# PFLeget/treegp

Measured on AMD Instinct MI355X. Metric: GP solve+predict throughput, 2-D AnisotropicRBF N=65536, higher is better.
Workload: dtype f64

## Files before the change

### include/tgp.h

```cpp
#ifndef TGP_H
#define TGP_H

#include <stdint.h>

#ifdef __cplusplus
extern "C" {
#endif

typedef struct tgp_ctx tgp_ctx;
typedef struct tgp_factor tgp_factor;

enum {
    TGP_RBF = 0,
    TGP_ARBF = 1,
    TGP_VK = 2,
    TGP_AVK = 3
};

typedef struct {
    int32_t kind;
    int32_t _pad;
    double amp;
    double a, b, c;
    double ell;
// ... 143 lines not shown
int tgp_dd_update2(tgp_ctx *ctx, double *d_Aloc, const int64_t *d_loff, int64_t Np, int kpanel, int G, int g,
                   const double *d_gathered0, int cmax0, const double *d_gathered1, int cmax1, int col_lo,
                   int col_hi);
int tgp_dd_update_group(tgp_ctx *ctx, double *d_Aloc, const int64_t *d_loff, int64_t Np, int kpanel, int G, int g,
                        int nseg, const double *const *d_gathered, const int *cmax, int col_lo, int col_hi);
int tgp_dd_strip_left(tgp_ctx *ctx, double *d_Aloc, const int64_t *h_loff, const int64_t *d_loff, int64_t Np, int kgroup, int b,
                      int G, int g, const double *d_ext);
int tgp_dd_queue_reset(tgp_ctx *ctx);
int tgp_dd_set_exclusive(tgp_ctx *ctx, int on);
int tgp_dd_update_group_queued(tgp_ctx *ctx, double *d_Aloc, const int64_t *d_loff, int64_t Np, int kpanel, int G, int g,
                               int nseg, const double *const *d_gathered, const int *cmax, int col_lo, int col_hi, int nres);
int tgp_dd_update_group_fused(tgp_ctx *ctx, double *d_Aloc, const int64_t *d_loff, int64_t Np, int kpanel, int G, int g, int nseg,
                              const double *const *d_gathered, const int *cmax, int head_cols, int nres);
int tgp_dd_wait_head(tgp_ctx *ctx, tgp_ctx *waiter);
int tgp_dd_tail_assemble(tgp_ctx *ctx, const double *d_gathered, int64_t stride, int64_t Np, int k0, int G, double *d_tail);
int tgp_dd_tail_scatter(tgp_ctx *ctx, const double *d_tail, int64_t Np, int k0, int G, int g, double *d_Aloc, const int64_t *d_loff);
int tgp_handoff_mode(tgp_ctx *ctx);
int tgp_dd_keep_panel(tgp_ctx *ctx, double *d_Afull, int64_t Np, int kpanel, int G, const double *d_bcast,
                      const double *d_gathered, int cmax);
int tgp_dd_fwd_diag(tgp_ctx *ctx, const double *d_Aloc, const int64_t *h_loff, int kb, const double *d_W, double *d_yk);
int tgp_dd_fwd_update(tgp_ctx *ctx, const double *d_Aloc, const int64_t *h_loff, int64_t Np, int kb, int G, int g,
                      const double *d_zk, double *d_yloc);
int tgp_dd_bwd_partial(tgp_ctx *ctx, const double *d_Aloc, const int64_t *h_loff, int64_t Np, int kb, int G, int g,
                       const double *d_aloc, double *d_s);
int tgp_dd_bwd_diag(tgp_ctx *ctx, const double *d_Aloc, const int64_t *h_loff, int kb, const double *d_W, double *d_ak,
                    const double *d_s );
int tgp_dd_logdet_local(tgp_ctx *ctx, const double *d_Aloc, const int64_t *d_loff, int64_t Np, int64_t n, int G, int g,
                        double *d_out);
int tgp_dd_info(tgp_ctx *ctx, int reset);

int tgp_debug_syrk_loop(tgp_ctx *ctx, double *d_A, int64_t Np, int reps, double *ms_per_launch,
                        double *flops_per_launch);
int tgp_debug_tilemap(int64_t T, int32_t *ti, int32_t *tj, int64_t cap);

#ifdef __cplusplus
}
#endif
#endif
```

### treegp_amd/_lib.py

```python
import ctypes as C
import os
import threading

import numpy as np

_HERE = os.path.dirname(os.path.abspath(__file__))
LIB_PATH = os.environ.get("TGP_LIB_PATH") or os.path.join(_HERE, "csrc", "libtgp.so")

TGP_RBF, TGP_ARBF, TGP_VK, TGP_AVK = 0, 1, 2, 3
NTIMINGS = 12


class TgpKernel(C.Structure):
    _fields_ = [("kind", C.c_int32), ("_pad", C.c_int32), ("amp", C.c_double), ("a", C.c_double),
                ("b", C.c_double), ("c", C.c_double), ("ell", C.c_double)]


_dp = C.POINTER(C.c_double)
_vp = C.c_void_p
_i64 = C.c_int64

SIGNATURES = {
    "tgp_init": (C.c_int, [C.POINTER(C.c_int), C.c_int, C.POINTER(_vp)]),
    "tgp_destroy": (None, [_vp]),
# ... 25 lines not shown
    "tgp_d2h": (C.c_int, [_vp, _vp, _vp, _i64]),
    "tgp_sync": (C.c_int, [_vp]),
    "tgp_stream": (_vp, [_vp]),
    "tgp_mem_info": (C.c_int, [_vp, C.POINTER(_i64), C.POINTER(_i64)]),
    "tgp_d_gp_solve": (C.c_int, [_vp, C.POINTER(TgpKernel), _vp, _i64, _vp, _vp, _vp, _dp, _dp, C.POINTER(_vp)]),
    "tgp_d_gp_predict": (C.c_int, [_vp, C.POINTER(TgpKernel), _vp, _i64, _vp, _vp, _i64, _vp]),
    "tgp_d_gp_predict_grad": (C.c_int, [_vp, C.POINTER(TgpKernel), _vp, _i64, _vp, _vp, _i64, _vp]),
    "tgp_panel_off": (_i64, [_i64, _i64]),
    "tgp_panel_elems": (_i64, [_i64]),
    "tgp_padded_n": (_i64, [_i64]),
    "tgp_d_kbuild_lower": (C.c_int, [_vp, C.POINTER(TgpKernel), _vp, _i64, _vp, _vp]),
    "tgp_d_potrf": (C.c_int, [_vp, _vp, _i64, _vp]),
    "tgp_d_potrs": (C.c_int, [_vp, _vp, _vp, _i64, _vp]),
    "tgp_d_potrs_multi": (C.c_int, [_vp, _vp, _vp, _i64, _vp, C.c_int]),
    "tgp_gp_solve_dense": (C.c_int, [_vp, _vp, _i64, _vp, _vp, _vp, _dp, _dp, C.POINTER(_vp)]),
    "tgp_d_gp_solve_dense": (C.c_int, [_vp, _vp, _i64, _vp, _vp, _vp, _dp, _dp, C.POINTER(_vp)]),
    "tgp_factor_solve": (C.c_int, [_vp, _vp, _vp, C.c_int, _vp]),
    "tgp_factor_lmul": (C.c_int, [_vp, _vp, _vp, C.c_int, _vp]),
    "tgp_factor_inv_diag": (C.c_int, [_vp, _vp, _vp]),
    "tgp_factor_inv_blocks": (C.c_int, [_vp, _vp, _vp, _i64, _vp]),
    "tgp_gp_solve_batch": (C.c_int, [_vp, C.c_int, _vp, _vp, _i64, _vp, _vp, _vp, _vp, _vp, _vp, _vp]),
    "tgp_gp_solve_grad_batch": (C.c_int, [_vp, C.c_int, _vp, _vp, _i64, _vp, _vp, _vp, _vp, _vp, _vp, _vp]),
    "tgp_gp_loo_batch": (C.c_int, [_vp, C.c_int, _vp, _vp, _i64, _vp, _vp, _vp, _vp, _vp, _vp, _vp, _vp]),
    "tgp_gp_posterior_batch": (C.c_int, [_vp, C.c_int, _vp, _vp, _i64, _vp, _vp, _vp, _vp, _i64, _vp, C.c_int, _vp, _vp, _vp, _vp, _vp]),
    "tgp_gp_predict_cov_dense": (C.c_int, [_vp, _vp, _vp, _vp, _i64, _vp]),
    "tgp_gp_predict_var": (C.c_int, [_vp, _vp, C.POINTER(TgpKernel), _vp, _i64, _vp, _i64, _vp]),
    "tgp_gp_predict_var_dense": (C.c_int, [_vp, _vp, _vp, _vp, _i64, _vp]),
    "tgp_gp_loglik_grad": (C.c_int, [_vp, _vp, C.POINTER(TgpKernel), _vp, _i64, _vp, _vp]),
    "tgp_d_gp_solve_grad": (C.c_int, [_vp, C.POINTER(TgpKernel), _vp, _i64, _vp, _vp, _dp, _dp, _vp]),
    "tgp_d_unpack_lower": (C.c_int, [_vp, _vp, _i64, _i64, _vp]),
    "tgp_factor_device": (C.c_int, [_vp, _vp, C.POINTER(_vp), C.POINTER(_vp), C.POINTER(_i64)]),
    "tgp_debug_syrk_loop": (C.c_int, [_vp, _vp, _i64, C.c_int, _dp, _dp]),
    "tgp_debug_tilemap": (C.c_int, [_i64, _vp, _vp, _i64]),
    "tgp_set_stream": (C.c_int, [_vp, _vp]),
    "tgp_reset_stream": (C.c_int, [_vp]),
    "tgp_set_side_stream": (C.c_int, [_vp, _vp]),
    "tgp_dist_panel_rows": (_i64, [_i64, _i64, C.c_int, C.c_int]),
    "tgp_dist_panel_off": (_i64, [_i64, _i64, C.c_int, C.c_int]),
    "tgp_dist_local_elems": (_i64, [_i64, C.c_int, C.c_int]),
    "tgp_dd_kbuild": (C.c_int, [_vp, C.POINTER(TgpKernel), _vp, _i64, _vp, _vp, _vp, C.c_int, C.c_int]),
    "tgp_dd_factor_diag": (C.c_int, [_vp, _vp, _vp, _i64, C.c_int, C.c_int, C.c_int, _vp, _vp]),
    "tgp_dd_trsm": (C.c_int, [_vp, _vp, _vp, _i64, C.c_int, C.c_int, C.c_int, _vp, _vp]),
    "tgp_dd_update": (C.c_int, [_vp, _vp, _vp, _i64, C.c_int, C.c_int, C.c_int, _vp, C.c_int, C.c_int, C.c_int]),
    "tgp_dd_update2": (C.c_int, [_vp, _vp, _vp, _i64, C.c_int, C.c_int, C.c_int, _vp, C.c_int, _vp, C.c_int, C.c_int, C.c_int]),
    "tgp_dd_update_group": (C.c_int, [_vp, _vp, _vp, _i64, C.c_int, C.c_int, C.c_int, C.c_int, _vp, _vp, C.c_int, C.c_int]),
    "tgp_dd_strip_left": (C.c_int, [_vp, _vp, _vp, _vp, _i64, C.c_int, C.c_int, C.c_int, C.c_int, _vp]),
    "tgp_dd_update_group_queued": (C.c_int, [_vp, _vp, _vp, _i64, C.c_int, C.c_int, C.c_int, C.c_int, _vp, _vp, C.c_int, C.c_int, C.c_int]),
    "tgp_dd_update_group_fused": (C.c_int, [_vp, _vp, _vp, _i64, C.c_int, C.c_int, C.c_int, C.c_int, _vp, _vp, C.c_int, C.c_int]),
    "tgp_dd_wait_head": (C.c_int, [_vp, _vp]),
    "tgp_handoff_mode": (C.c_int, [_vp]),
    "tgp_dd_tail_assemble": (C.c_int, [_vp, _vp, _i64, _i64, C.c_int, C.c_int, _vp]),
    "tgp_dd_tail_scatter": (C.c_int, [_vp, _vp, _i64, C.c_int, C.c_int, C.c_int, _vp, _vp]),
    "tgp_dd_queue_reset": (C.c_int, [_vp]),
    "tgp_dd_set_exclusive": (C.c_int, [_vp, C.c_int]),
    "tgp_dd_keep_panel": (C.c_int, [_vp, _vp, _i64, C.c_int, C.c_int, _vp, _vp, C.c_int]),
    "tgp_dd_fwd_diag": (C.c_int, [_vp, _vp, _vp, C.c_int, _vp, _vp]),
    "tgp_dd_fwd_update": (C.c_int, [_vp, _vp, _vp, _i64, C.c_int, C.c_int, C.c_int, _vp, _vp]),
    "tgp_dd_bwd_partial": (C.c_int, [_vp, _vp, _vp, _i64, C.c_int, C.c_int, C.c_int, _vp, _vp]),
    "tgp_dd_bwd_diag": (C.c_int, [_vp, _vp, _vp, C.c_int, _vp, _vp, _vp]),
    "tgp_dd_logdet_local": (C.c_int, [_vp, _vp, _vp, _i64, _i64, C.c_int, C.c_int, _vp]),
    "tgp_dd_info": (C.c_int, [_vp, C.c_int]),
}

_lib = None
_ctx = {}
_lock = threading.Lock()
# ... 135 lines not shown
```

### treegp_amd/csrc/chol.hip

```cpp
#include "tgp_internal.h"

#include "gemm_tile.h"
#include "potrf128.h"

#ifdef TGP_POTRF_STAMPS
__device__ unsigned long long tgp_gemm_stamps[1024 * 4];
__device__ int tgp_gemm_stamp_grid = 43;
__device__ unsigned long long tgp_queue_stamps[1024 * 4];
__device__ int tgp_queue_stamp_T = 40;
__device__ unsigned long long tgp_mid_stamps[25 * 8];
__device__ int tgp_mid_stamp_base = 5120;
#define TGP_MID_STAMP(i)                                                                                   \
    do {                                                                                                   \
        if (threadIdx.x == 0 && base == tgp_mid_stamp_base && blockIdx.x < 25) tgp_mid_stamps[blockIdx.x * 8 + (i)] = __builtin_amdgcn_s_memrealtime(); \
    } while (0)
#else
#define TGP_MID_STAMP(i) ((void)0)
#endif

namespace {
template <int MODE, int LDB>
__global__ __launch_bounds__(256, 2) void gemm_col_kernel(const double *A, const double *B, double *C) {
    const int64_t t = blockIdx.x;
    TGP_CHAIN_PRIO();
// ... 151 lines not shown
    const int ri = blockIdx.x;
    const int tj = blockIdx.y;
    if (tj > (ri >> 3) || (ri >> 3) >= T) return;
    TGP_CHAIN_PRIO();
    const int64_t pj = ob + (tj >> 1);
    const int64_t I = (int64_t)TGP_PW * ob + 16 * (int64_t)ri;
    double *C = Abase + panel_off(pj, Np) + (I - pj * TGP_PW) * TGP_PW + (tj & 1) * TGP_TB;
    const int64_t oa = (int64_t)ri * 16 * TGP_PW, obb = (int64_t)tj * TGP_TB * TGP_PW;
    nt_slice_tile<1, TGP_PW, NSEG>(nt_slice_lds_storage(), P0 + oa, TGP_PW, P0 + obb, TGP_PW, C, TGP_PW, NSEG > 1 ? P1 + oa : nullptr,
                                   NSEG > 1 ? P1 + obb : nullptr);
}

template <int NSEG>
__global__ __launch_bounds__(256, 2) void syrk_dtv_kernel(double *Abase, int64_t Np, int ob, int T, int strip, const double *P0,
                                                          const double *P1) {
    int ti, tj;
    if (strip == 0) {
        tilemap(blockIdx.x, T, ti, tj);
        if (ti < 0) return;
    } else {
        tj = (int)(blockIdx.x % strip);
        ti = (int)(blockIdx.x / strip);
        if (ti < tj || ti >= T) return;
    }
    if (strip) TGP_CHAIN_PRIO();
    const int64_t pj = ob + (tj >> 1);
    const int64_t I = (int64_t)TGP_PW * ob + (int64_t)TGP_TB * ti;
    double *C = Abase + panel_off(pj, Np) + (I - pj * TGP_PW) * TGP_PW + (tj & 1) * TGP_TB;
    const int64_t oa = (int64_t)ti * TGP_TB * TGP_PW, obb = (int64_t)tj * TGP_TB * TGP_PW;
    gemm_tile_dtv<4, TGP_PW, NSEG>(P0 + oa, P0 + obb, C, NSEG > 1 ? P1 + oa : nullptr, NSEG > 1 ? P1 + obb : nullptr);
}

template <int NSEG>
__global__ __launch_bounds__(256, 2) void syrk_strip64_kernel(double *Abase, int64_t Np, int ob, int T, int strip, const double *P0,
                                                              const double *P1, int ti_min = 0) {
    const int tj = (int)(blockIdx.x % strip);
    const int th = (int)(blockIdx.x / strip) + 2 * ti_min;
    const int ti = th >> 1;
    if (ti < tj || ti >= T) return;
    TGP_CHAIN_PRIO();
    const int64_t pj = ob + (tj >> 1);
    const int64_t I = (int64_t)TGP_PW * ob + (int64_t)64 * th;
    double *C = Abase + panel_off(pj, Np) + (I - pj * TGP_PW) * TGP_PW + (tj & 1) * TGP_TB;
    const int64_t oa = (int64_t)th * 64 * TGP_PW, obb = (int64_t)tj * TGP_TB * TGP_PW;
    gemm_tile_dtv<4, TGP_PW, NSEG, 1>(P0 + oa, P0 + obb, C, NSEG > 1 ? P1 + oa : nullptr, NSEG > 1 ? P1 + obb : nullptr);
}

template <int NSEG>
__global__ __launch_bounds__(256, 2) void syrk_strip32_kernel(double *Abase, int64_t Np, int ob, int T, int strip, const double *P0,
                                                              const double *P1) {
    const int tj = (int)(blockIdx.x % strip);
    const int tq = (int)(blockIdx.x / strip);
    const int ti = tq >> 2;
    if (ti < tj || ti >= T) return;
    TGP_CHAIN_PRIO();
    const int64_t pj = ob + (tj >> 1);
    const int64_t I = (int64_t)TGP_PW * ob + (int64_t)32 * tq;
    double *C = Abase + panel_off(pj, Np) + (I - pj * TGP_PW) * TGP_PW + (tj & 1) * TGP_TB;
    const int64_t oa = (int64_t)tq * 32 * TGP_PW, obb = (int64_t)tj * TGP_TB * TGP_PW;
    gemm_tile_dtv32<TGP_PW, NSEG>(P0 + oa, P0 + obb, C, NSEG > 1 ? P1 + oa : nullptr, NSEG > 1 ? P1 + obb : nullptr);
}

template <int NSEG>
__global__ __launch_bounds__(256, 2) void syrk_dtv_queue_kernel(double *Abase, int64_t Np, int ob, int T, unsigned entries, unsigned half_from, int nres,
                                                                unsigned *__restrict__ queue, const double *P0, const double *P1, int steal) {
    __shared__ unsigned s_slot;
// ... 67 lines not shown
#endif
    }
}

struct HeadSignal {
    unsigned *done = nullptr, *flag = nullptr;
    unsigned target = 0, seq = 0;
    int nhead = 0;
};
__device__ __forceinline__ void head_done(const HeadSignal &h) {
    asm volatile("s_waitcnt vmcnt(0)" ::: "memory");
    __syncthreads();
    if (threadIdx.x < 64) {
        __builtin_amdgcn_fence(__ATOMIC_RELEASE, "agent");
        if (threadIdx.x == 0) {
            const unsigned old = __hip_atomic_fetch_add(h.done, 1u, __ATOMIC_ACQ_REL, __HIP_MEMORY_SCOPE_AGENT);
            if (old + 1u == h.target) __hip_atomic_store(h.flag, h.seq, __ATOMIC_RELEASE, __HIP_MEMORY_SCOPE_SYSTEM);
        }
    }
}

template <int NSEG>
__global__ __launch_bounds__(256, 2) void syrk_segs_kernel(double *Abase, int64_t Np, int ob, int T, int strip, SegPtrs<NSEG> P) {
    int ti, tj;
    if (strip == 0) {
        tilemap(blockIdx.x, T, ti, tj);
        if (ti < 0) return;
    } else {
        tj = (int)(blockIdx.x % strip);
        ti = (int)(blockIdx.x / strip);
        if (ti < tj || ti >= T) return;
    }
    if (strip) TGP_CHAIN_PRIO();
    const int64_t pj = ob + (tj >> 1);
    const int64_t I = (int64_t)TGP_PW * ob + (int64_t)TGP_TB * ti;
    double *C = Abase + panel_off(pj, Np) + (I - pj * TGP_PW) * TGP_PW + (tj & 1) * TGP_TB;
    const int64_t oa = (int64_t)ti * TGP_TB * TGP_PW, obb = (int64_t)tj * TGP_TB * TGP_PW;
    SegPtrs<NSEG> sp;
#pragma unroll
    for (int s = 0; s < NSEG; ++s) {
        sp.a[s] = P.a[s] + oa;
        sp.b[s] = P.a[s] + obb;
    }
    gemm_tile_dtv_segs<4, TGP_PW, NSEG>(sp, C);
}

template <int NSEG>
struct DistSegs {
    const double *P[NSEG];
    const double *PB[NSEG];
    int cmax[NSEG];
    int frg[NSEG];
};
struct DistMap {
    int start[258];
    int ngroups;
    int qfb;
    unsigned ginv;
    int whole;
    int half_from;
    int nhead, head_cols;
    int head_half;
    HeadSignal hs;
};
__device__ __forceinline__ int div_g(int x, unsigned ginv) { return ginv ? (int)__umulhi((unsigned)x, ginv) : x; }
__device__ __forceinline__ int snake_pos(int q, int r, int G) { return (q & 1) ? G - 1 - r : r; }
// ... 163 lines not shown
        gemm_col_small_kernel<0, TGP_TB><<<8, 256, 0, st>>>(R1, W0, R1);
        if (r2 > 0) {
            if (small) gemm_col_small_kernel<0, TGP_TB><<<r2 * 8, 256, 0, st>>>(R2, W0, R2);
            else gemm_col_kernel<0, TGP_TB><<<r2, 256, 0, st>>>(R2, W0, R2);
        }
        gemm_col_small_kernel<1, TGP_PW><<<8, 256, 0, st>>>(R1, R1, R1 + TGP_TB);
        if (r2 > 0) {
            if (small) gemm_col_small_kernel<1, TGP_PW><<<r2 * 8, 256, 0, st>>>(R2, R1, R2 + TGP_TB);
            else gemm_col_kernel<1, TGP_PW><<<r2, 256, 0, st>>>(R2, R1, R2 + TGP_TB);
        }
        run_potrf128(st, R1 + TGP_TB, TGP_PW, W1, d_info, base + TGP_TB, exclusive, solo);
    } else {
        if (r1 <= small_rows) {
            gemm_col_small_kernel<0, TGP_TB><<<r1 * 8, 256, 0, st>>>(R1, W0, R1);
            gemm_col_small_kernel<1, TGP_PW><<<r1 * 8, 256, 0, st>>>(R1, R1, R1 + TGP_TB);
        } else {
            gemm_col_kernel<0, TGP_TB><<<r1, 256, 0, st>>>(R1, W0, R1);
            gemm_col_kernel<1, TGP_PW><<<r1, 256, 0, st>>>(R1, R1, R1 + TGP_TB);
        }
        run_potrf128(st, R1 + TGP_TB, TGP_PW, W1, d_info, base + TGP_TB, exclusive, solo);
    }
    if (r2 > 0) {
        double *R2 = Pk + (int64_t)TGP_PW * TGP_PW + TGP_TB;
        if (r2 <= small_rows) gemm_col_small_kernel<0, TGP_TB><<<r2 * 8, 256, 0, st>>>(R2, W1, R2);
        else gemm_col_kernel<0, TGP_TB><<<r2, 256, 0, st>>>(R2, W1, R2);
    }
}

inline int small_t() {
    static const int v = [] { const char *e = getenv("TGP_SMALL_T"); return e ? atoi(e) : 8; }();
    return v;
}

template <int NSEG>
void launch_syrk(hipStream_t st, double *d_A, int64_t Np, int ob, int T, int strip, const double *P0, const double *P1) {
    if (T <= 0) return;
    static const int strip_small_t = [] { const char *e = getenv("TGP_STRIP_SMALL_T"); return e ? atoi(e) : 16; }();
    if (T <= small_t() || (strip > 0 && T <= strip_small_t)) {
        const int cols = strip == 0 ? T : (strip < T ? strip : T);
        syrk_small_kernel<NSEG><<<dim3((unsigned)(T * 8), (unsigned)cols), 256, 0, st>>>(d_A, Np, ob, T, P0, P1);
        return;
    }
    static const int strip64_t = [] { const char *e = getenv("TGP_STRIP64_T"); return e ? atoi(e) : 128; }();
    static const int strip32_t = [] { const char *e = getenv("TGP_STRIP32_T"); return e ? atoi(e) : 64; }();
    if (strip > 0 && T <= strip32_t) {
        syrk_strip32_kernel<NSEG><<<(unsigned)((int64_t)4 * T * strip), 256, 0, st>>>(d_A, Np, ob, T, strip, P0, P1);
        return;
    }
    if (strip > 0 && T <= strip64_t) {
        syrk_strip64_kernel<NSEG><<<(unsigned)((int64_t)2 * T * strip), 256, 0, st>>>(d_A, Np, ob, T, strip, P0, P1);
        return;
    }
    const unsigned gs = strip == 0 ? (unsigned)tilemap_grid(T) : (unsigned)((int64_t)T * strip);
    syrk_dtv_kernel<NSEG><<<gs, 256, 0, st>>>(d_A, Np, ob, T, strip, P0, P1);
}

int queued_nres(int T) {
    static const int queue_res = [] { const char *e = getenv("TGP_QUEUE_RES"); return e ? atoi(e) : 0; }();
    if (queue_res > 0) return queue_res > TGP_QUEUE_MAXRES ? TGP_QUEUE_MAXRES : queue_res;
    static const int t1 = [] { const char *e = getenv("TGP_QUEUE_T1"); return e ? atoi(e) : 42; }();
    static const int t2 = [] { const char *e = getenv("TGP_QUEUE_T2"); return e ? atoi(e) : 26; }();
    return T >= t1 ? 1 : (T >= t2 ? 2 : 3);
}
void launch_syrk2_queued(tgp_ctx *ctx, hipStream_t st, double *d_A, int64_t Np, int ob, int T, const double *P0, const double *P1,
                         int nqueue) {
    const int nres = queued_nres(T);
    static const int half_env = [] { const char *e = getenv("TGP_QUEUE_HALF"); return e ? atoi(e) : -1; }();
    const unsigned slots = (unsigned)(tilemap_grid(T) / 8);
    unsigned nhalf = half_env >= 0 ? (unsigned)half_env : (unsigned)(512 - 64 * nres) / 8u;
    if (nhalf > slots) nhalf = slots;
    static const int steal = [] { const char *e = getenv("TGP_QUEUE_STEAL"); return e ? atoi(e) : 1; }();
    syrk_dtv_queue_kernel<2><<<512 + 8, 256, 0, st>>>(d_A, Np, ob, T, slots + nhalf, slots - nhalf, nres,
                                                     ctx->d_queue + TGP_QUEUE_WORDS * nqueue, P0, P1, steal);
}
}

int launch_potrf(tgp_ctx *ctx, double *d_A, int64_t Np, double *d_W, bool defer_info, int64_t n_data) {
    TGP_ARG(Np > 0 && Np % TGP_PW == 0);
    hipStream_t st = ctx->stream;
    TGP_HIP(hipMemsetAsync(ctx->d_info, 0, sizeof(int), st));
    const int nP = (int)(Np / TGP_PW);
    const bool prof = ctx->profiling != 0;
    if (prof) {
        while ((int)ctx->prof_events.size() < 2 * nP) {
            hipEvent_t e;
            TGP_HIP(hipEventCreate(&e));
// ... 22 lines not shown
        return 0;
    };
    auto Wk = [&](int k) { return d_W + (int64_t)(2 * k) * TGP_TB * TGP_TB; };
    auto panel = [&](int k) { return d_A + panel_off(k, Np); };
    static const int queue_t = [] { const char *e = getenv("TGP_QUEUE_T"); return e ? atoi(e) : 64; }();
    int nqueue = 0;
    static const bool mid_env = [] { const char *e = getenv("TGP_PANEL_MID"); return e ? atoi(e) != 0 : true; }();
    const bool mid_on = mid_env && !ctx->mid_off && ctx->mid_allowed;
    if (mid_on) TGP_HIP(hipMemsetAsync(ctx->d_psync, 0, (size_t)(nP < TGP_PSYNC_PANELS ? nP : TGP_PSYNC_PANELS) * PANEL_SYNC_WORDS * sizeof(unsigned), st));
    if (Np / TGP_TB - 8 > small_t())
        TGP_HIP(hipMemsetAsync(ctx->d_queue, 0, TGP_NQUEUE * TGP_QUEUE_WORDS * sizeof(unsigned), st));
    auto psync = [&](int k) { return (mid_on && k < TGP_PSYNC_PANELS) ? ctx->d_psync + PANEL_SYNC_WORDS * k : nullptr; };
    auto run_pairs = [&](int kstart) -> int {
        hipStream_t sd = ctx->side_stream;
        auto factor_pair = [&](hipStream_t s, int k, bool exclusive = false, int cus = 0, bool tell = false) {
            const int64_t mk = Np - (int64_t)TGP_PW * k;
            auto sync = [&](int kk) { return (cus > 0 && mid_on && kk < TGP_PSYNC_PANELS) ? ctx->d_psync + PANEL_SYNC_WORDS * kk : nullptr; };
            factor_panel(s, panel(k), mk, Wk(k), ctx->d_info, k * TGP_PW, exclusive, n_data, sync(k), cus);
            if (tell) (void)tgp_signal(ctx, s, 2, ctx->ev[6]);
            if (k + 1 >= nP) return;
            const int T1 = (int)((mk - TGP_PW) / TGP_TB);
            launch_syrk<1>(s, d_A, Np, k + 1, T1, 2, panel(k) + (int64_t)TGP_PW * TGP_PW, nullptr);
            factor_panel(s, panel(k + 1), mk - TGP_PW, Wk(k + 1), ctx->d_info, (k + 1) * TGP_PW, exclusive, n_data, sync(k + 1), cus);
        };
        factor_pair(st, kstart, false, 256);
        static const int split_t = [] { const char *e = getenv("TGP_U2A_SPLIT_T"); return e ? atoi(e) : 64; }();
        bool early = false;
        for (int k = kstart; k + 2 < nP; k += 2) {
            const int T2 = (int)((Np - (int64_t)TGP_PW * (k + 2)) / TGP_TB);
            const double *P0 = panel(k) + (int64_t)2 * TGP_PW * TGP_PW;
            const double *P1 = panel(k + 1) + (int64_t)TGP_PW * TGP_PW;
            const int T3 = T2 - 4;
            const bool queued = T3 <= queue_t && T3 > small_t() && nqueue < TGP_NQUEUE;
            {
                const double rows = (double)T2 * TGP_TB, w = (T2 < 4 ? T2 : 4) * (double)TGP_TB;
                const double elems = w * (rows - w) + w * (w + 1.0) / 2.0;
                int rc = timed([&] {
                    if (early) launch_syrk<1>(st, d_A, Np, k + 2, T2, 4, P1, nullptr);
                    else launch_syrk<2>(st, d_A, Np, k + 2, T2, 4, P0, P1);
                }, (early ? 1.0 : 2.0) * 2.0 * TGP_PW * elems);
                if (rc) return rc;
            }
            TGP_HIP(tgp_signal(ctx, st, 0, ctx->ev[4]));
            TGP_HIP(tgp_await(ctx, sd, 0, ctx->ev[4]));
            const bool early_next = T3 > 0 && T3 <= split_t;
            factor_pair(sd, k + 2, queued, queued ? 32 * queued_nres(T3) : (T3 <= small_t() ? 256 : 0), early_next);
            TGP_HIP(tgp_signal(ctx, sd, 1, ctx->ev[5]));
            if (T3 > 0) {
                const double m = (double)T3 * TGP_TB;
                const int64_t skip = (int64_t)4 * TGP_TB * TGP_PW;
                int rc = timed([&] {
                    if (queued) launch_syrk2_queued(ctx, st, d_A, Np, k + 4, T3, P0 + skip, P1 + skip, nqueue++);
                    else launch_syrk<2>(st, d_A, Np, k + 4, T3, 0, P0 + skip, P1 + skip);
                }, 2.0 * TGP_PW * m * (m + 1.0));
                if (rc) return rc;
            }
            if (early_next) {
                TGP_HIP(tgp_await(ctx, st, 2, ctx->ev[6]));
                launch_syrk<1>(st, d_A, Np, k + 4, T3, 4, panel(k + 2) + (int64_t)2 * TGP_PW * TGP_PW, nullptr);
            }
            early = early_next;
            TGP_HIP(tgp_await(ctx, st, 1, ctx->ev[5]));
        }
        return 0;
    };
    if (mode == 0) {
        for (int k = 0; k < nP; ++k) {
            const int64_t mk = Np - (int64_t)TGP_PW * k;
            factor_panel(st, panel(k), mk, Wk(k), ctx->d_info, k * TGP_PW, false, n_data, psync(k), 256);
            const int T = (int)((mk - TGP_PW) / TGP_TB);
            if (T > 0) {
                const double m = (double)T * TGP_TB;
                int rc = timed([&] { launch_syrk<1>(st, d_A, Np, k + 1, T, 0, panel(k) + (int64_t)TGP_PW * TGP_PW, nullptr); },
                               (double)TGP_PW * m * (m + 1.0));
                if (rc) return rc;
            }
        }
    } else if (mode == 3) {
        hipStream_t sd = ctx->side_stream;
        auto seg_rows = [&](int kpanel, int first_block) {
            return (const double *)(panel(kpanel) + (int64_t)(first_block - kpanel) * TGP_PW * TGP_PW);
        };
        auto strip_update = [&](hipStream_t s, int k0, int j) {
            const int ob = k0 + j;
            const int T = (int)((Np - (int64_t)TGP_PW * ob) / TGP_TB);
            if (T <= small_t()) {
                for (int i = 0; i < j; ++i)
                    syrk_small_kernel<1><<<dim3((unsigned)(T * 8), 2u), 256, 0, s>>>(d_A, Np, ob, T, seg_rows(k0 + i, ob), nullptr);
                return;
            }
            const unsigned gs = (unsigned)((int64_t)T * 2);
            if (j == 1) {
                SegPtrs<1> P{{seg_rows(k0, ob)}, {nullptr}};
                syrk_segs_kernel<1><<<gs, 256, 0, s>>>(d_A, Np, ob, T, 2, P);
            } else if (j == 2) {
                SegPtrs<2> P{{seg_rows(k0, ob), seg_rows(k0 + 1, ob)}, {nullptr, nullptr}};
                syrk_segs_kernel<2><<<gs, 256, 0, s>>>(d_A, Np, ob, T, 2, P);
            } else {
                SegPtrs<3> P{{seg_rows(k0, ob), seg_rows(k0 + 1, ob), seg_rows(k0 + 2, ob)}, {nullptr, nullptr, nullptr}};
                syrk_segs_kernel<3><<<gs, 256, 0, s>>>(d_A, Np, ob, T, 2, P);
            }
        };
        auto factor_group = [&](hipStream_t s, int k0) {
            for (int j = 0; j < 4 && k0 + j < nP; ++j) {
                if (j > 0) strip_update(s, k0, j);
                factor_panel(s, panel(k0 + j), Np - (int64_t)TGP_PW * (k0 + j), Wk(k0 + j), ctx->d_info, (k0 + j) * TGP_PW, false, n_data);
            }
        };
        auto bulk = [&](int k0, int ob, int T, int strip) {
            if (T <= small_t()) {
                const int cols = strip == 0 ? T : (strip < T ? strip : T);
                for (int i = 0; i < 4; i += 2)
                    syrk_small_kernel<2><<<dim3((unsigned)(T * 8), (unsigned)cols), 256, 0, st>>>(
                        d_A, Np, ob, T, seg_rows(k0 + i, ob), seg_rows(k0 + i + 1, ob));
                return;
            }
            SegPtrs<4> P{{seg_rows(k0, ob), seg_rows(k0 + 1, ob), seg_rows(k0 + 2, ob), seg_rows(k0 + 3, ob)},
                         {nullptr, nullptr, nullptr, nullptr}};
            const unsigned gs = strip == 0 ? (unsigned)tilemap_grid(T) : (unsigned)((int64_t)T * strip);
            syrk_segs_kernel<4><<<gs, 256, 0, st>>>(d_A, Np, ob, T, strip, P);
        };
        static const int tail_tiles = [] { const char *e = getenv("TGP_QUAD_TAIL_TILES"); return e ? atoi(e) : 96; }();
        factor_group(st, 0);
        for (int k = 0; k + 4 < nP; k += 4) {
            const int T4 = (int)((Np - (int64_t)TGP_PW * (k + 4)) / TGP_TB);
            if (T4 <= tail_tiles) {
                const double m = (double)T4 * TGP_TB;
                int rc = timed([&] { bulk(k, k + 4, T4, 0); }, 4.0 * TGP_PW * m * (m + 1.0));
                if (rc) return rc;
                counting = false;
                rc = run_pairs(k + 4);
                counting = true;
                if (rc) return rc;
                break;
            }
            {
                const double rows = (double)T4 * TGP_TB, w = (T4 < 8 ? T4 : 8) * (double)TGP_TB;
                const double elems = w * (rows - w) + w * (w + 1.0) / 2.0;
                int rc = timed([&] { bulk(k, k + 4, T4, 8); }, 2.0 * 4.0 * TGP_PW * elems);
                if (rc) return rc;
            }
            TGP_HIP(tgp_signal(ctx, st, 0, ctx->ev[4]));
            TGP_HIP(tgp_await(ctx, sd, 0, ctx->ev[4]));
            factor_group(sd, k + 4);
            TGP_HIP(tgp_signal(ctx, sd, 1, ctx->ev[5]));
            const int T5 = T4 - 8;
            if (T5 > 0) {
                const double m = (double)T5 * TGP_TB;
                int rc = timed([&] { bulk(k, k + 8, T5, 0); }, 4.0 * TGP_PW * m * (m + 1.0));
                if (rc) return rc;
            }
            TGP_HIP(tgp_await(ctx, st, 1, ctx->ev[5]));
        }
    } else if (mode == 2) {
        int rc = run_pairs(0);
        if (rc) return rc;
    } else {
        for (int k = 0; k < nP; k += 2) {
            const int64_t mk = Np - (int64_t)TGP_PW * k;
            factor_panel(st, panel(k), mk, Wk(k), ctx->d_info, k * TGP_PW, false, n_data, psync(k), 256);
            if (k + 1 >= nP) break;
            const int T1 = (int)((mk - TGP_PW) / TGP_TB);
            launch_syrk<1>(st, d_A, Np, k + 1, T1, 2, panel(k) + (int64_t)TGP_PW * TGP_PW, nullptr);
            factor_panel(st, panel(k + 1), mk - TGP_PW, Wk(k + 1), ctx->d_info, (k + 1) * TGP_PW, false, n_data, psync(k + 1), 256);
            const int T2 = T1 - 2;
            if (T2 > 0) {
                const double m = (double)T2 * TGP_TB;
                int rc = timed([&] { launch_syrk<2>(st, d_A, Np, k + 2, T2, 0, panel(k) + (int64_t)2 * TGP_PW * TGP_PW,
                                                     panel(k + 1) + (int64_t)TGP_PW * TGP_PW); },
                               2.0 * TGP_PW * m * (m + 1.0));
                if (rc) return rc;
            }
        }
    }
    TGP_HIP(hipGetLastError());
    TGP_HIP(hipMemcpyAsync(ctx->h_info, ctx->d_info, sizeof(int), hipMemcpyDeviceToHost, st));
    ctx->timings[6] = nlaunch;
    ctx->timings[7] = flops;
    ctx->timings[5] = 0.0;
    if (defer_info && !prof) return 0;
    TGP_HIP(hipStreamSynchronize(st));
    if (prof) {
// ... 182 lines not shown

#ifdef TGP_POTRF_STAMPS
extern "C" int tgp_debug_gemm_stamps(unsigned long long *out, int grid) {
    if (grid > 0) return (int)hipMemcpyToSymbol(HIP_SYMBOL(tgp_gemm_stamp_grid), &grid, sizeof(int));
    return (int)hipMemcpyFromSymbol(out, HIP_SYMBOL(tgp_gemm_stamps), 1024 * 4 * sizeof(unsigned long long));
}
extern "C" int tgp_debug_queue_stamps(unsigned long long *out, int T) {
    if (T > 0) return (int)hipMemcpyToSymbol(HIP_SYMBOL(tgp_queue_stamp_T), &T, sizeof(int));
    return (int)hipMemcpyFromSymbol(out, HIP_SYMBOL(tgp_queue_stamps), 1024 * 4 * sizeof(unsigned long long));
}
extern "C" int tgp_debug_mid_stamps(unsigned long long *out, int base) {
    if (base >= 0) return (int)hipMemcpyToSymbol(HIP_SYMBOL(tgp_mid_stamp_base), &base, sizeof(int));
    return (int)hipMemcpyFromSymbol(out, HIP_SYMBOL(tgp_mid_stamps), 25 * 8 * sizeof(unsigned long long));
}
extern "C" int tgp_debug_potrf_fine(unsigned long long *out) {
    return (int)hipMemcpyFromSymbol(out, HIP_SYMBOL(tgp_potrf_fine), 1024 * 8 * sizeof(unsigned long long));
}
extern "C" int tgp_debug_potrf_stamps(unsigned long long *out) {
    return (int)hipMemcpyFromSymbol(out, HIP_SYMBOL(tgp_potrf_stamps), 1024 * 20 * sizeof(unsigned long long));
}
#endif

int tgp_debug_tilemap(int64_t T, int32_t *ti, int32_t *tj, int64_t cap) {
    const int64_t g = tilemap_grid(T);
    if (cap < g) return -1;
    for (int64_t b = 0; b < g; ++b) {
        int i, j;
        tilemap(b, T, i, j);
        ti[b] = i;
        tj[b] = j;
    }
    return (int)g;
}
```

### treegp_amd/csrc/tgp_internal.h

```cpp
#pragma once
#include <hip/hip_runtime.h>
#include <cstdint>
#include <cstdio>
#include <cstdlib>
#include <cstring>
#include <string>
#include <atomic>
#include <vector>
#include "../../include/tgp.h"

#ifdef TGP_NO_CHAIN_PRIO
#define TGP_CHAIN_PRIO() ((void)0)
#else
#define TGP_CHAIN_PRIO() __builtin_amdgcn_s_setprio(3)
#endif

#define TGP_QUEUE_MAXRES 6
#define TGP_QUEUE_LEAVE (8 + 32 * TGP_QUEUE_MAXRES)
#define TGP_QUEUE_WORDS (TGP_QUEUE_LEAVE + 8)
#define TGP_NQUEUE 128
#define TGP_PSYNC_PANELS 1024
#define TGP_TB 128
#define TGP_PW 256
#define TGP_VAR_CHUNK_MAX 65280
// ... 107 lines not shown
    const int64_t S = (T + (1 << sh) - 1) >> sh;
    const int64_t ns = S * (S + 1) / 2;
    const int64_t per = (int64_t)1 << (2 * sh), q = per >= 8 ? per / 8 : 1;
    return (ns / 8) * per + (ns % 8) * q;
}
__host__ __device__ inline int64_t tilemap_grid(int64_t T) { return 8 * tilemap_slots(T); }
__host__ __device__ inline void tilemap(int64_t b, int64_t T, int &ti, int &tj) {
    ti = -1; tj = -1;
    if (T <= 0 || b < 0) return;
    const int sh = tilemap_sup_shift(T);
    const int64_t S = (T + (1 << sh) - 1) >> sh;
    const int64_t ns = S * (S + 1) / 2;
    const int per = 1 << (2 * sh), q = per >= 8 ? per / 8 : 1;
    const int xcd = (int)(b & 7);
    const int64_t slot = b >> 3;
    const int64_t whole = (ns / 8) * per;
    int64_t st;
    int within;
    if (slot < whole) {
        st = (slot >> (2 * sh)) * 8 + xcd;
        within = (int)(slot & (per - 1));
    } else {
        const int64_t nn = slot - whole;
        st = (ns / 8) * 8 + nn / q;
        within = xcd * q + (int)(nn % q);
        if (st >= ns || within >= per) return;
    }
    int64_t Si, Sj;
    tri_index(st, Si, Sj);
    const int i = (int)((Si << sh) + (within >> sh));
    const int j = (int)((Sj << sh) + (within & ((1 << sh) - 1)));
    if (j > i || i >= T) return;
    ti = i; tj = j;
}

int tgp_ensure_side_stream(tgp_ctx *ctx);
int tgp_ensure_scratch(tgp_ctx *ctx, size_t bytes);
int tgp_ensure_scratch2(tgp_ctx *ctx, size_t bytes);
int tgp_ensure_pinned(tgp_ctx *ctx, size_t bytes, void **out);
int launch_kbuild_lower(tgp_ctx *ctx, const tgp_kernel *k, const double *d_X, int64_t n, int64_t Np,
                        const double *d_yerr, double *d_A);
int launch_kernel_dense(tgp_ctx *ctx, const tgp_kernel *k, const double *d_X, int64_t n,
                        const double *d_Y, int64_t m, int self, double *d_out);
int launch_potrf(tgp_ctx *ctx, double *d_A, int64_t Np, double *d_W, bool defer_info = false, int64_t n_data = -1);
int tgp_potrf_info_rc(tgp_ctx *ctx, int info);
#define TGP_RC_HANDOFF (-4)
extern std::atomic<int> tgp_solves_in_flight;
#define TGP_FLAG_HEAD 8
#define TGP_FLAG_HEAD_COUNT 9
bool tgp_handoff_by_flags(tgp_ctx *ctx);
unsigned tgp_next_seq(tgp_ctx *ctx, int id, hipError_t *err);
hipError_t tgp_signal_value(tgp_ctx *ctx, hipStream_t from, int id, unsigned v);
hipError_t tgp_signal(tgp_ctx *ctx, hipStream_t from, int id, hipEvent_t ev);
hipError_t tgp_await(tgp_ctx *ctx, hipStream_t to, int id, hipEvent_t ev);
bool potrs_big_step(int64_t Np, int *S);
int acquire_slabs(tgp_ctx *ctx, int64_t Np, int S, double **slab_cache, int *slab_S, double **out, bool *need_build);
int launch_potrs_big_bwd(tgp_ctx *ctx, const double *d_A, int64_t Np, int S, const double *slabs, double *d_b, double *d_z);
int launch_kbuild_lower_dist(tgp_ctx *ctx, const tgp_kernel *k, const double *d_X, int64_t n, int64_t Np,
                             const double *d_yerr, double *d_Aloc, const int64_t *d_loff, int G, int g);
int launch_factor_diag256(tgp_ctx *ctx, double *blk, double *W0, double *W1, int base, bool latency = false);
int launch_trsm_rows(tgp_ctx *ctx, double *rows, int ntiles, const double *Lkk, const double *W0, const double *W1, double *keepW = nullptr);
int launch_syrk_distn(tgp_ctx *ctx, double *d_Aloc, const int64_t *d_loff, int64_t Np, int kpanel, int G, int g, int nseg,
                      const double *const *d_P, const int *cmax, int col_lo, int col_hi, int queue_nres = 0, int head_cols = 0,
                      const double *const *d_PB = nullptr);
int launch_diag256_fwd(tgp_ctx *ctx, const double *Lkk, const double *W0, const double *W1, double *y);
int launch_diag256_bwd(tgp_ctx *ctx, const double *Lkk, const double *W0, const double *W1, double *y, const double *s);
// ... 41 lines not shown
```

Baseline: 243,800.

## Pad strip SYRK head launch with trailing bulk tiles to fill waves

The strip (lookahead) SYRK launch now uses a head kernel whose grid is rounded up to a multiple of 256 blocks. The padding blocks compute the last tiles of the following bulk trailing update, and the bulk launch shrinks its grid by the same amount. This is meant to fill the partial wave of the latency-critical strip launch with useful work and shorten the bulk launch. The risk is correctness and ordering: the filler tiles must not depend on the strip results, and a debug mapping export is added to check this.

```diff
diff --git a/include/tgp.h b/include/tgp.h
--- a/include/tgp.h
+++ b/include/tgp.h
@@ -199,6 +199,8 @@
 int tgp_debug_syrk_loop(tgp_ctx *ctx, double *d_A, int64_t Np, int reps, double *ms_per_launch,
                         double *flops_per_launch);
 int tgp_debug_tilemap(int64_t T, int32_t *ti, int32_t *tj, int64_t cap);
+int tgp_debug_head_split(int64_t T, int strip, int64_t *info, int32_t *head_ti, int32_t *head_tj, int32_t *head_slot,
+                         int32_t *bulk_ti, int32_t *bulk_tj, int64_t cap);
 
 #ifdef __cplusplus
 }
diff --git a/treegp_amd/_lib.py b/treegp_amd/_lib.py
--- a/treegp_amd/_lib.py
+++ b/treegp_amd/_lib.py
@@ -81,6 +81,7 @@
     "tgp_factor_device": (C.c_int, [_vp, _vp, C.POINTER(_vp), C.POINTER(_vp), C.POINTER(_i64)]),
     "tgp_debug_syrk_loop": (C.c_int, [_vp, _vp, _i64, C.c_int, _dp, _dp]),
     "tgp_debug_tilemap": (C.c_int, [_i64, _vp, _vp, _i64]),
+    "tgp_debug_head_split": (C.c_int, [_i64, C.c_int, _vp, _vp, _vp, _vp, _vp, _vp, _i64]),
     "tgp_set_stream": (C.c_int, [_vp, _vp]),
     "tgp_reset_stream": (C.c_int, [_vp]),
     "tgp_set_side_stream": (C.c_int, [_vp, _vp]),
diff --git a/treegp_amd/csrc/chol.hip b/treegp_amd/csrc/chol.hip
--- a/treegp_amd/csrc/chol.hip
+++ b/treegp_amd/csrc/chol.hip
@@ -207,6 +207,21 @@
 }
 
 template <int NSEG>
+__global__ __launch_bounds__(256, 2) void syrk_dtv_head_kernel(double *Abase, int64_t Np, int ob, int T, int strip, int need, int fill,
+                                                               const double *P0, const double *P1) {
+    int ti, tj;
+    bool filler;
+    head_tile(blockIdx.x, T, strip, need, fill, ti, tj, filler);
+    if (ti < 0) return;
+    if (!filler) TGP_CHAIN_PRIO();
+    const int64_t pj = ob + (tj >> 1);
+    const int64_t I = (int64_t)TGP_PW * ob + (int64_t)TGP_TB * ti;
+    double *C = Abase + panel_off(pj, Np) + (I - pj * TGP_PW) * TGP_PW + (tj & 1) * TGP_TB;
+    const int64_t oa = (int64_t)ti * TGP_TB * TGP_PW, obb = (int64_t)tj * TGP_TB * TGP_PW;
+    gemm_tile_dtv<4, TGP_PW, NSEG>(P0 + oa, P0 + obb, C, NSEG > 1 ? P1 + oa : nullptr, NSEG > 1 ? P1 + obb : nullptr);
+}
+
+template <int NSEG>
 __global__ __launch_bounds__(256, 2) void syrk_strip64_kernel(double *Abase, int64_t Np, int ob, int T, int strip, const double *P0,
                                                               const double *P1, int ti_min = 0) {
     const int tj = (int)(blockIdx.x % strip);
@@ -340,6 +355,27 @@
         if (ti < tj || ti >= T) return;
     }
     if (strip) TGP_CHAIN_PRIO();
+    const int64_t pj = ob + (tj >> 1);
+    const int64_t I = (int64_t)TGP_PW * ob + (int64_t)TGP_TB * ti;
+    double *C = Abase + panel_off(pj, Np) + (I - pj * TGP_PW) * TGP_PW + (tj & 1) * TGP_TB;
+    const int64_t oa = (int64_t)ti * TGP_TB * TGP_PW, obb = (int64_t)tj * TGP_TB * TGP_PW;
+    SegPtrs<NSEG> sp;
+#pragma unroll
+    for (int s = 0; s < NSEG; ++s) {
+        sp.a[s] = P.a[s] + oa;
+        sp.b[s] = P.a[s] + obb;
+    }
+    gemm_tile_dtv_segs<4, TGP_PW, NSEG>(sp, C);
+}
+
+template <int NSEG>
+__global__ __launch_bounds__(256, 2) void syrk_segs_head_kernel(double *Abase, int64_t Np, int ob, int T, int strip, int need, int fill,
+                                                                SegPtrs<NSEG> P) {
+    int ti, tj;
+    bool filler;
+    head_tile(blockIdx.x, T, strip, need, fill, ti, tj, filler);
+    if (ti < 0) return;
+    if (!filler) TGP_CHAIN_PRIO();
     const int64_t pj = ob + (tj >> 1);
     const int64_t I = (int64_t)TGP_PW * ob + (int64_t)TGP_TB * ti;
     double *C = Abase + panel_off(pj, Np) + (I - pj * TGP_PW) * TGP_PW + (tj & 1) * TGP_TB;
@@ -569,26 +605,58 @@
     return v;
 }
 
-template <int NSEG>
-void launch_syrk(hipStream_t st, double *d_A, int64_t Np, int ob, int T, int strip, const double *P0, const double *P1) {
+inline int strip_small_t() {
+    static const int v = [] { const char *e = getenv("TGP_STRIP_SMALL_T"); return e ? atoi(e) : 16; }();
+    return v;
+}
+inline int strip32_t() {
+    static const int v = [] { const char *e = getenv("TGP_STRIP32_T"); return e ? atoi(e) : 64; }();
+    return v;
+}
+inline int strip64_t() {
+    static const int v = [] { const char *e = getenv("TGP_STRIP64_T"); return e ? atoi(e) : 128; }();
+    return v;
+}
+inline bool strip_on_full_tile(int T) { return T > small_t() && T > strip_small_t() && T > strip32_t() && T > strip64_t(); }
+
+inline bool head_fill_on() {
+    static const bool v = [] { const char *e = getenv("TGP_HEAD_FILL"); return e ? atoi(e) != 0 : true; }();
+    return v;
+}
+inline HeadSplit head_split_for(int T, int strip) { return head_fill_on() ? head_split(T, strip, small_t()) : HeadSplit(); }
+inline double head_fill_flops(const HeadSplit &h, int T, int strip, double depth) {
+    double elems = 0.0;
+    for (int i = 0; i < h.fill; ++i) {
+        int ti, tj;
+        bool filler;
+        head_tile((int64_t)h.need + i, T, strip, h.need, h.fill, ti, tj, filler);
+        if (ti >= 0) elems += ti == tj ? TGP_TB * (TGP_TB + 1.0) / 2.0 : (double)TGP_TB * TGP_TB;
+    }
+    return 2.0 * depth * elems;
+}
+
+template <int NSEG>
+void launch_syrk(hipStream_t st, double *d_A, int64_t Np, int ob, int T, int strip, const double *P0, const double *P1,
+                 const HeadSplit &split = HeadSplit()) {
     if (T <= 0) return;
-    static const int strip_small_t = [] { const char *e = getenv("TGP_STRIP_SMALL_T"); return e ? atoi(e) : 16; }();
-    if (T <= small_t() || (strip > 0 && T <= strip_small_t)) {
+    if (T <= small_t() || (strip > 0 && T <= strip_small_t())) {
         const int cols = strip == 0 ? T : (strip < T ? strip : T);
         syrk_small_kernel<NSEG><<<dim3((unsigned)(T * 8), (unsigned)cols), 256, 0, st>>>(d_A, Np, ob, T, P0, P1);
         return;
     }
-    static const int strip64_t = [] { const char *e = getenv("TGP_STRIP64_T"); return e ? atoi(e) : 128; }();
-    static const int strip32_t = [] { const char *e = getenv("TGP_STRIP32_T"); return e ? atoi(e) : 64; }();
-    if (strip > 0 && T <= strip32_t) {
+    if (strip > 0 && T <= strip32_t()) {
         syrk_strip32_kernel<NSEG><<<(unsigned)((int64_t)4 * T * strip), 256, 0, st>>>(d_A, Np, ob, T, strip, P0, P1);
         return;
     }
-    if (strip > 0 && T <= strip64_t) {
+    if (strip > 0 && T <= strip64_t()) {
         syrk_strip64_kernel<NSEG><<<(unsigned)((int64_t)2 * T * strip), 256, 0, st>>>(d_A, Np, ob, T, strip, P0, P1);
         return;
     }
-    const unsigned gs = strip == 0 ? (unsigned)tilemap_grid(T) : (unsigned)((int64_t)T * strip);
+    if (strip > 0 && split.need > 0) {
+        syrk_dtv_head_kernel<NSEG><<<(unsigned)(split.need + split.fill), 256, 0, st>>>(d_A, Np, ob, T, strip, split.need, split.fill, P0, P1);
+        return;
+    }
+    const unsigned gs = strip == 0 ? (unsigned)(tilemap_grid(T) - split.fill) : (unsigned)((int64_t)T * strip);
     syrk_dtv_kernel<NSEG><<<gs, 256, 0, st>>>(d_A, Np, ob, T, strip, P0, P1);
 }
 
@@ -677,13 +745,15 @@
             const double *P1 = panel(k + 1) + (int64_t)TGP_PW * TGP_PW;
             const int T3 = T2 - 4;
             const bool queued = T3 <= queue_t && T3 > small_t() && nqueue < TGP_NQUEUE;
+            const HeadSplit split = (!early && !queued && strip_on_full_tile(T2)) ? head_split_for(T2, 4) : HeadSplit();
+            const double fill_flops = head_fill_flops(split, T2, 4, 2.0 * TGP_PW);
             {
                 const double rows = (double)T2 * TGP_TB, w = (T2 < 4 ? T2 : 4) * (double)TGP_TB;
                 const double elems = w * (rows - w) + w * (w + 1.0) / 2.0;
                 int rc = timed([&] {
                     if (early) launch_syrk<1>(st, d_A, Np, k + 2, T2, 4, P1, nullptr);
-                    else launch_syrk<2>(st, d_A, Np, k + 2, T2, 4, P0, P1);
-                }, (early ? 1.0 : 2.0) * 2.0 * TGP_PW * elems);
+                    else launch_syrk<2>(st, d_A, Np, k + 2, T2, 4, P0, P1, split);
+                }, (early ? 1.0 : 2.0) * 2.0 * TGP_PW * elems + fill_flops);
                 if (rc) return rc;
             }
             TGP_HIP(tgp_signal(ctx, st, 0, ctx->ev[4]));
@@ -696,8 +766,8 @@
                 const int64_t skip = (int64_t)4 * TGP_TB * TGP_PW;
                 int rc = timed([&] {
                     if (queued) launch_syrk2_queued(ctx, st, d_A, Np, k + 4, T3, P0 + skip, P1 + skip, nqueue++);
-                    else launch_syrk<2>(st, d_A, Np, k + 4, T3, 0, P0 + skip, P1 + skip);
-                }, 2.0 * TGP_PW * m * (m + 1.0));
+                    else launch_syrk<2>(st, d_A, Np, k + 4, T3, 0, P0 + skip, P1 + skip, split);
+                }, 2.0 * TGP_PW * m * (m + 1.0) - fill_flops);
                 if (rc) return rc;
             }
             if (early_next) {
@@ -752,7 +822,7 @@
                 factor_panel(s, panel(k0 + j), Np - (int64_t)TGP_PW * (k0 + j), Wk(k0 + j), ctx->d_info, (k0 + j) * TGP_PW, false, n_data);
             }
         };
-        auto bulk = [&](int k0, int ob, int T, int strip) {
+        auto bulk = [&](int k0, int ob, int T, int strip, const HeadSplit &split = HeadSplit()) {
             if (T <= small_t()) {
                 const int cols = strip == 0 ? T : (strip < T ? strip : T);
                 for (int i = 0; i < 4; i += 2)
@@ -762,7 +832,11 @@
             }
             SegPtrs<4> P{{seg_rows(k0, ob), seg_rows(k0 + 1, ob), seg_rows(k0 + 2, ob), seg_rows(k0 + 3, ob)},
                          {nullptr, nullptr, nullptr, nullptr}};
-            const unsigned gs = strip == 0 ? (unsigned)tilemap_grid(T) : (unsigned)((int64_t)T * strip);
+            if (strip > 0 && split.need > 0) {
+                syrk_segs_head_kernel<4><<<(unsigned)(split.need + split.fill), 256, 0, st>>>(d_A, Np, ob, T, strip, split.need, split.fill, P);
+                return;
+            }
+            const unsigned gs = strip == 0 ? (unsigned)(tilemap_grid(T) - split.fill) : (unsigned)((int64_t)T * strip);
             syrk_segs_kernel<4><<<gs, 256, 0, st>>>(d_A, Np, ob, T, strip, P);
         };
         static const int tail_tiles = [] { const char *e = getenv("TGP_QUAD_TAIL_TILES"); return e ? atoi(e) : 96; }();
@@ -779,10 +853,12 @@
                 if (rc) return rc;
                 break;
             }
+            const HeadSplit split = T4 > small_t() ? head_split_for(T4, 8) : HeadSplit();
+            const double fill_flops = head_fill_flops(split, T4, 8, 4.0 * TGP_PW);
             {
                 const double rows = (double)T4 * TGP_TB, w = (T4 < 8 ? T4 : 8) * (double)TGP_TB;
                 const double elems = w * (rows - w) + w * (w + 1.0) / 2.0;
-                int rc = timed([&] { bulk(k, k + 4, T4, 8); }, 2.0 * 4.0 * TGP_PW * elems);
+                int rc = timed([&] { bulk(k, k + 4, T4, 8, split); }, 2.0 * 4.0 * TGP_PW * elems + fill_flops);
                 if (rc) return rc;
             }
             TGP_HIP(tgp_signal(ctx, st, 0, ctx->ev[4]));
@@ -792,7 +868,7 @@
             const int T5 = T4 - 8;
             if (T5 > 0) {
                 const double m = (double)T5 * TGP_TB;
-                int rc = timed([&] { bulk(k, k + 8, T5, 0); }, 4.0 * TGP_PW * m * (m + 1.0));
+                int rc = timed([&] { bulk(k, k + 8, T5, 0, split); }, 4.0 * TGP_PW * m * (m + 1.0) - fill_flops);
                 if (rc) return rc;
             }
             TGP_HIP(tgp_await(ctx, st, 1, ctx->ev[5]));
@@ -1041,3 +1117,28 @@
     }
     return (int)g;
 }
+
+int tgp_debug_head_split(int64_t T, int strip, int64_t *info, int32_t *head_ti, int32_t *head_tj, int32_t *head_slot,
+                         int32_t *bulk_ti, int32_t *bulk_tj, int64_t cap) {
+    if (T <= 0 || T > (1 << 20) || strip <= 0 || strip > 64) return -1;
+    const HeadSplit h = head_split_for((int)T, strip);
+    const int need = head_need((int)T, strip);
+    const int64_t hg = need + h.fill, bg = tilemap_grid(T - strip) - h.fill;
+    if (cap < hg || cap < bg) return -1;
+    info[0] = need; info[1] = h.fill; info[2] = hg; info[3] = bg;
+    for (int64_t b = 0; b < hg; ++b) {
+        int i, j;
+        bool filler;
+        head_tile(b, (int)T, strip, need, h.fill, i, j, filler);
+        head_ti[b] = i;
+        head_tj[b] = j;
+        head_slot[b] = filler ? (int32_t)(bg + (b - need)) : -1;
+    }
+    for (int64_t b = 0; b < bg; ++b) {
+        int i, j;
+        tilemap(b, T - strip, i, j);
+        bulk_ti[b] = i < 0 ? -1 : i + strip;
+        bulk_tj[b] = i < 0 ? -1 : j + strip;
+    }
+    return 0;
+}
diff --git a/treegp_amd/csrc/tgp_internal.h b/treegp_amd/csrc/tgp_internal.h
--- a/treegp_amd/csrc/tgp_internal.h
+++ b/treegp_amd/csrc/tgp_internal.h
@@ -163,6 +163,43 @@
     const int j = (int)((Sj << sh) + (within & ((1 << sh) - 1)));
     if (j > i || i >= T) return;
     ti = i; tj = j;
+}
+
+struct HeadSplit {
+    int need = 0;
+    int fill = 0;
+};
+__host__ __device__ inline int head_need(int T, int strip) {
+    const int w = T < strip ? T : strip;
+    return w * (w + 1) / 2 + (T - w) * w;
+}
+__host__ __device__ inline HeadSplit head_split(int T, int strip, int min_bulk_T) {
+    HeadSplit h;
+    h.need = head_need(T, strip);
+    const int fill = (256 - h.need % 256) % 256;
+    if (T - strip > min_bulk_T && fill < tilemap_grid(T - strip)) h.fill = fill;
+    return h;
+}
+__host__ __device__ inline void head_tile(int64_t b, int T, int strip, int need, int fill, int &ti, int &tj, bool &filler) {
+    filler = b >= need;
+    if (!filler) {
+        const int w = T < strip ? T : strip, tri = w * (w + 1) / 2;
+        if (b < tri) {
+            int i = 0;
+            while ((i + 1) * (i + 2) / 2 <= b) ++i;
+            ti = i;
+            tj = (int)b - i * (i + 1) / 2;
+        } else {
+            ti = strip + (int)((b - tri) / strip);
+            tj = (int)((b - tri) % strip);
+        }
+        return;
+    }
+    tilemap(tilemap_grid(T - strip) - fill + (b - need), T - strip, ti, tj);
+    if (ti >= 0) {
+        ti += strip;
+        tj += strip;
+    }
 }
 
 int tgp_ensure_side_stream(tgp_ctx *ctx);
```

Result: no change. 244,300 (median of 6 runs) (+0.2%).
